# AchilleBailly/zstd-decompressor

Measured on AMD Instinct MI355X. Metric: decompressed MB/s (bit-exact vs ref) + % HBM roofline, higher is better.
Workload: dtype u8; 1 GPU; C4: enwik-style text, 128 KiB frames, zstd -3, 1 GiB unique x10 = one 10 GiB corpus; frames_total=81920, frames_rank0=81920, decompressed_bytes_total=10737418240, decompressed_bytes_rank0=10737418240, compressed_bytes_rank0=4645362830, sequences_rank0=1186360140, parallelism=replicas x1, step=zd_decode_async over every resident frame, launched per step

## Files before the change

### zstd-decompressor_amd/csrc/zd_kernels.hip

```cpp
#include <hip/hip_runtime.h>
#include <stddef.h>
#include <stdint.h>
#include <type_traits>

#include "../../include/zd.h"
#include "zd_chain.h"
#include "zd_common.h"
#include "zd_huf.h"
#include "zd_launch.h"
#include "zd_walk.h"

namespace zd {

const char* const kKernelNames[N_KERNELS] = {"zd_k_rawcopy", "zd_k_tables", "zd_k_huffman", "zd_k_sequences",
                                             "zd_k_execute", "zd_k_jexec"};
const char* const kDomNames[N_DOM] = {"zd_k_rawcopy", "zd_k_fused", "zd_k_execute", "zd_k_execute_lds",
                                      "zd_k_jsum+zd_k_jsum_blocks+zd_k_jprefix+zd_k_jscatter+zd_k_jround"};

__constant__ uint32_t c_ml_base[53] = {
    3,  4,  5,  6,  7,  8,  9,  10, 11, 12, 13, 14, 15, 16, 17, 18, 19, 20, 21, 22, 23, 24, 25, 26, 27, 28, 29,
    30, 31, 32, 33, 34, 35, 37, 39, 41, 43, 47, 51, 59, 67, 83, 99, 131, 259, 515, 1027, 2051, 4099, 8195, 16387, 32771, 65539};
__constant__ uint8_t c_ml_bits[53] = {0, 0, 0, 0, 0, 0, 0, 0, 0, 0, 0, 0, 0, 0, 0, 0, 0, 0, 0, 0, 0, 0, 0, 0, 0, 0, 0,
                                      0, 0, 0, 0, 0, 1, 1, 1, 1, 2, 2, 3, 3, 4, 4, 5, 7, 8, 9, 10, 11, 12, 13, 14, 15, 16};
__constant__ uint32_t c_ll_base[36] = {0,  1,  2,  3,  4,  5,  6,   7,   8,   9,   10,   11,   12,   13,   14,   15,   16,    18,
// ... 1504 lines not shown
                                                           uint32_t n_list, const uint16_t* __restrict__ fses,
                                                           uint64_t* __restrict__ recs) {
  __shared__ __attribute__((aligned(16))) uint16_t tabs[K3_LANES * K3_TAB];
  const int lane = threadIdx.x;
  const uint32_t li = blockIdx.x * K3_LANES + lane;
  bool act = li < n_list;
  const uint32_t ci = act ? list[li] : 0;
  CompBlock C;
  if (act) C = comp[ci];
  if (act) {
    const uint64_t key0 = fstate[C.frame].key;
    if (key0 != KEY_NONE && key_phase(key0) == PH_PARSE) act = false;
  }
  int al[3] = {0, 0, 0};
  const uint16_t* g[3] = {nullptr, nullptr, nullptr};
  if (act) {
    for (int k = 0; k < 3; k++) {
      const uint32_t s = (uint32_t)C.tab_src[k];
      al[k] = cstate[s].al[k];
      g[k] = fses + (uint64_t)comp[s].fse_slot * FSE_SLOT + k * FSE_TAB;
    }
  }
  const bool deep = act && al[1] > 8;
  const bool use_lds = __ballot(deep) == 0;
  lds_u16* mine = (lds_u16*)tabs + lane * K3_TAB;
  if (use_lds && act) {
    const int dst[3] = {0, K3_TL + K3_TM, K3_TL};
    for (int k = 0; k < 3; k++) {
      const int cnt = 1 << al[k];
      if (cnt >= 8) {
        typedef uint32_t u32x4 __attribute__((ext_vector_type(4)));
        typedef __attribute__((address_space(1))) const u32x4 g_u4;
        typedef __attribute__((address_space(3))) u32x4 l_u4;
        g_u4* s4 = (g_u4*)g[k];
        l_u4* d4 = (l_u4*)(mine + dst[k]);
        for (int e = 0; e < cnt / 8; e++) {
          u32x4 v = s4[e];
          v.x = K3_ENTRY(v.x & 0xFFFF, k, al[k]) | (K3_ENTRY(v.x >> 16, k, al[k]) << 16);
          v.y = K3_ENTRY(v.y & 0xFFFF, k, al[k]) | (K3_ENTRY(v.y >> 16, k, al[k]) << 16);
          v.z = K3_ENTRY(v.z & 0xFFFF, k, al[k]) | (K3_ENTRY(v.z >> 16, k, al[k]) << 16);
          v.w = K3_ENTRY(v.w & 0xFFFF, k, al[k]) | (K3_ENTRY(v.w >> 16, k, al[k]) << 16);
          d4[e] = v;
        }
      } else {
        for (int e = 0; e < cnt; e++) mine[dst[k] + e] = (uint16_t)K3_ENTRY(((g_u16*)g[k])[e], k, al[k]);
      }
    }
  }
  __syncthreads();
  if (!act) return;
  const CompState cs = cstate[ci];
  const uint8_t* blk = src + C.src;
  const uintptr_t lo = (uintptr_t)src;
  int st = 0;
  bool exact = !use_lds;
  if (use_lds)
    exact = K3_FAST(blk + cs.bs_off, cs.bs_size, lo, mine, mine + K3_TL, mine + K3_TL + K3_TM, al[0], al[1],
                       al[2], C.nseq, recs + C.seq_out) != 0;
  if (exact)
    st = K3_CHAIN<g_u16*, true>(blk + cs.bs_off, cs.bs_size, lo, (g_u16*)g[0], (g_u16*)g[2], (g_u16*)g[1], al[0],
                                 al[1], al[2], C.nseq, recs + C.seq_out);
  if (st) k3_fail(C, ci, cstate, fstate, st);
}
template <int CTRL>
__device__ inline uint32_t qdpp(uint32_t x) {
  return (uint32_t)__builtin_amdgcn_mov_dpp((int)x, CTRL, 0xf, 0xf, false);
}
constexpr int QP_SWAP1 = 0xB1;
constexpr int QP_SWAP2 = 0x4E;
__device__ inline uint32_t quad_sum(uint32_t x) {
  x += qdpp<QP_SWAP1>(x);
  return x + qdpp<QP_SWAP2>(x);
}
__device__ inline uint32_t quad_or(uint32_t x) {
  x |= qdpp<QP_SWAP1>(x);
  return x | qdpp<QP_SWAP2>(x);
}
__device__ inline uint32_t quad_max(uint32_t x) {
  x = max(x, qdpp<QP_SWAP1>(x));
  return max(x, qdpp<QP_SWAP2>(x));
}
template <int L, int N, bool PUB = false>
__device__ int seq_chainq(const uint8_t* bs, uint32_t bs_size, uintptr_t base, const lds_u16* tab, int role,
                          int all, int alo, int alm, uint32_t n, uint64_t* __restrict__ out,
                          volatile __attribute__((address_space(3))) uint32_t* prog = nullptr) {
  constexpr int U = (L % 2 == 0) ? L : 2 * L;
  if (bs_size == 0) return 1;
  const uint8_t lastb = bs[bs_size - 1];
  if (lastb == 0) return 1;
  int32_t pos = (int32_t)(8 * (bs_size - 1)) + highbit32(lastb);
  const int32_t A = all + alo + alm;
  if (A > pos) return 1;
  if ((intptr_t)bs - (intptr_t)base + (intptr_t)bs_size < 4 * N) return 1;
  const int32_t m = (int32_t)max((intptr_t)base - (intptr_t)bs, (intptr_t)(-4 * N));
  const int32_t pos0 = pos;
  const Win6 wi = win6_load(bs, m, pos);
  const uint32_t v0 = win6_bits(wi, pos, (uint32_t)A);
  const int alr = role == 0 ? alo : role == 1 ? alm : all;
  const uint32_t m3 = role == 3 ? 0u : ~0u, m0 = role == 0 ? 0u : ~0u;
  const uint32_t ar = (uint32_t)(alr - 31), Tr = 1u << alr;
  uint32_t s = role == 0 ? __builtin_amdgcn_ubfe(v0, alm, alo)
             : role == 1 ? __builtin_amdgcn_ubfe(v0, 0, alm)
             : v0 >> (alo + alm);
  pos -= A;
  uint32_t pS = s, pPos = (uint32_t)pos;
  auto pair_word = [&](uint32_t sB, uint32_t posB) -> uint32_t {
    const uint32_t d = pS | (sB << 10);
    const uint32_t x = d | ((pPos - posB) << 20);
    return role == 3 ? pPos : (role == 0 ? x : d);
  };
  g_u32* const outw = (g_u32*)out + role;
  const uint32_t n_even = (n + 1) & ~1u;
  WinN<N> w[L];
#pragma unroll
  for (int k = 0; k < L; k++) {
    w[k] = winn_load<N>(bs, m, k == 0 ? pos0 : pos);
    if (!(k & 1)) {
      asm volatile("" ::: "memory");
      outw[0] = pair_word(s, (uint32_t)pos);
    }
  }
  uint32_t mx = 0;
  int32_t ymin = 0;
  auto step = [&](WinN<N>& use) {
    const uint32_t e = tab[s];
    mx = max(mx, e);
    const uint32_t ns = e & 1023, nb = __builtin_clz(ns) + ar;
    const uint32_t c = e >> 10;
    const uint32_t csum = qdpp<0x00>(c) + qdpp<0x55>(c) + qdpp<0xAA>(c);
    const int32_t y = (pos - use.wb) - (int32_t)csum;
    pos -= (int32_t)csum;
    ymin = min(ymin, y);
    const uint32_t r = winn_at_tree<N>(use, (uint32_t)y);
    use = winn_load<N>(bs, m, pos);
    const uint32_t t = qdpp<0x50>(nb) & m0;
    const uint32_t v = __builtin_amdgcn_ubfe(r, t + qdpp<0x50>(t), nb);
    s = (ns << nb) + v - Tr;
  };
  uint32_t i = 0;
  g_u32* wp = outw;
  for (; i + 1 < n; i += U) {
#pragma unroll
    for (int k = 0; k < U; k += 2) {
      step(w[k % L]);
      asm volatile("" ::: "memory");
      const uint32_t slot = i + k;
      if constexpr (U == 4) {
        *wp = pair_word(s, (uint32_t)pos);
        wp += 4;
      } else {
        outw[2 * (slot < n ? slot : n_even)] = pair_word(s, (uint32_t)pos);
      }
      if constexpr (PUB) {
        constexpr int K3_PAIR_VMEM = 2 * (N / 4 + (N % 4 == 2 ? 1 : 0)) + 1;
        static_assert(7 * K3_PAIR_VMEM > 32, "seq_chainq PUB: vmcnt(32) would not cover the published line's stores");
        if (((slot + 2) & 15) == 0 && slot + 2 >= 32) {
          asm volatile("s_waitcnt vmcnt(32)" ::: "memory");
          if (role == 0) *prog = (slot + 2 - 16) >> 4;
        }
      }
      step(w[(k + 1) % L]);
      pS = s;
      pPos = (uint32_t)pos;
    }
  }
  outw[2 * (i < n ? i : n_even)] = pair_word(pS, pPos);
  const uint64_t rl = k3_reread(out, n - 1);
  const int32_t pl = (int32_t)(uint32_t)rl;
  const uint32_t st = (uint32_t)(rl >> 32);
  const uint32_t shr = role == 0 ? 20 : role == 1 ? 10 : 0;
  const uint32_t el = tab[(st >> shr) & 1023] & m3;
  mx = quad_max(max(mx, el));
  const uint32_t S = quad_sum((__builtin_clz(el & 1023) + ar) & m3);
  const int32_t E = (int32_t)(quad_sum(el >> 10) - S);
  return (mx >= K3F_BAD || ymin < 0 || pl < 0 || E > pl) ? 1 : 0;
}

#ifndef ZD_K3H_RING
#define ZD_K3H_RING 3
#endif
#ifndef ZD_K3H_DELAY
#define ZD_K3H_DELAY 1
#endif
#ifndef ZD_K3H_BITS
#define ZD_K3H_BITS 26
#endif
template <int R, int D>
__device__ constexpr int k3h_reload(int t) {
  const int x = t - 1 - D + (t - 1 - D < 0 ? 2 * R : 0);
  return x % 2 == 0 ? (x / 2) % R : -1;
}
template <int R, int D, int N>
__device__ int seq_chainqh(const uint8_t* bs, uint32_t bs_size, uintptr_t base, const lds_u16* tab, int role,
                           int all, int alo, int alm, uint32_t n, uint64_t* __restrict__ out) {
  static_assert(R >= 2 && D >= 0 && D <= 2 * R - 4, "seq_chainqh: a slot is loaded at least a whole step before its use");
  constexpr int U = 2 * R;
  if (bs_size == 0) return 1;
  const uint8_t lastb = bs[bs_size - 1];
  if (lastb == 0) return 1;
  int32_t pos = (int32_t)(8 * (bs_size - 1)) + highbit32(lastb);
  const int32_t A = all + alo + alm;
  if (A > pos) return 1;
  if ((intptr_t)bs - (intptr_t)base + (intptr_t)bs_size < 4 * N) return 1;
  const int32_t m = (int32_t)max((intptr_t)base - (intptr_t)bs, (intptr_t)(-4 * N));
  const Win6 wi = win6_load(bs, m, pos);
  const uint32_t v0 = win6_bits(wi, pos, (uint32_t)A);
  const int alr = role == 0 ? alo : role == 1 ? alm : all;
  const uint32_t m3 = role == 3 ? 0u : ~0u, m0 = role == 0 ? 0u : ~0u;
  const uint32_t ar = (uint32_t)(alr - 31), Tr = 1u << alr;
  uint32_t s = role == 0 ? __builtin_amdgcn_ubfe(v0, alm, alo)
             : role == 1 ? __builtin_amdgcn_ubfe(v0, 0, alm)
             : v0 >> (alo + alm);
  pos -= A;
  uint32_t pS = s, pPos = (uint32_t)pos;
  auto pair_word = [&](uint32_t sB, uint32_t posB) -> uint32_t {
    const uint32_t d = pS | (sB << 10);
    const uint32_t x = d | ((pPos - posB) << 20);
    return role == 3 ? pPos : (role == 0 ? x : d);
  };
  g_u32* const outw = (g_u32*)out + role;
  const uint32_t n_even = (n + 1) & ~1u;
  WinN<N> w[R];
  w[0] = winn_load<N>(bs, m, pos);
  asm volatile("" ::: "memory");
  outw[0] = pair_word(s, (uint32_t)pos);
#pragma unroll
  for (int k = 1; k < R; k++) w[k] = w[0];
  uint32_t mx = 0;
  int32_t ymin = 0;
  auto step = [&](WinN<N>& use, WinN<N>* rl) {
    const uint32_t e = tab[s];
    mx = max(mx, e);
    const uint32_t ns = e & 1023, nb = __builtin_clz(ns) + ar;
    const uint32_t c = e >> 10;
    const uint32_t csum = qdpp<0x00>(c) + qdpp<0x55>(c) + qdpp<0xAA>(c);
    const int32_t y = (pos - use.wb) - (int32_t)csum;
    pos -= (int32_t)csum;
    ymin = min(ymin, y);
    uint32_t r = winn_at_tree<N>(use, (uint32_t)y);
    if (rl) {
      if (rl == &use) asm volatile("" : "+v"(r) : : "memory");
      *rl = winn_load<N>(bs, m, pos);
    }
    const uint32_t t = qdpp<0x50>(nb) & m0;
    const uint32_t v = __builtin_amdgcn_ubfe(r, t + qdpp<0x50>(t), nb);
    s = (ns << nb) + v - Tr;
  };
  uint32_t i = 0;
  g_u32* wp = outw;
  for (; i + 1 < n; i += U) {
#pragma unroll
    for (int k = 0; k < R; k++) {
      const int ra = k3h_reload<R, D>(2 * k), rb = k3h_reload<R, D>(2 * k + 1);
      step(w[k], ra >= 0 ? &w[ra] : nullptr);
      asm volatile("" ::: "memory");
      if (k < 2)
        wp[4 * k] = pair_word(s, (uint32_t)pos);
      else
        outw[2 * min(i + 2 * k, n_even)] = pair_word(s, (uint32_t)pos);
      step(w[k], rb >= 0 ? &w[rb] : nullptr);
      pS = s;
      pPos = (uint32_t)pos;
    }
    wp += 4 * R;
  }
  outw[2 * (i < n ? i : n_even)] = pair_word(pS, pPos);
  const uint64_t rl = k3_reread(out, n - 1);
  const int32_t pl = (int32_t)(uint32_t)rl;
  const uint32_t st = (uint32_t)(rl >> 32);
  const uint32_t shr = role == 0 ? 20 : role == 1 ? 10 : 0;
  const uint32_t el = tab[(st >> shr) & 1023] & m3;
  mx = quad_max(max(mx, el));
  const uint32_t S = quad_sum((__builtin_clz(el & 1023) + ar) & m3);
  const int32_t E = (int32_t)(quad_sum(el >> 10) - S);
  return (mx >= K3F_BAD || ymin < 0 || pl < 0 || E > pl) ? 1 : 0;
}

#ifdef ZD_K3_COUNT
__device__ unsigned long long zd_k3_count[4];
extern "C" int zd_debug_k3_count(unsigned long long* v, int reset) {
  if (hipMemcpyFromSymbol(v, HIP_SYMBOL(zd_k3_count), sizeof(zd_k3_count)) != hipSuccess) return -1;
  if (reset) {
    const unsigned long long z[4] = {0, 0, 0, 0};
    if (hipMemcpyToSymbol(HIP_SYMBOL(zd_k3_count), z, sizeof(z)) != hipSuccess) return -1;
  }
  return 0;
}
#endif

#ifndef ZD_K3Q_CHAINS
#define ZD_K3Q_CHAINS 16
#endif
constexpr int K3Q_CHAINS = ZD_K3Q_CHAINS;
static_assert(K3Q_CHAINS == 8 || K3Q_CHAINS == 16, "K3Q: 8 or 16 chains per wave");
__global__ __launch_bounds__(64) void zd_k_sequences_q(const uint8_t* __restrict__ src,
                                                       const CompBlock* __restrict__ comp, CompState* cstate,
                                                       FrameState* fstate, const uint32_t* __restrict__ list,
                                                       uint32_t n_list, const uint16_t* __restrict__ fses,
                                                       uint64_t* __restrict__ recs, const uint8_t* __restrict__ redo) {
  __shared__ __attribute__((aligned(16))) uint16_t tabs[K3Q_CHAINS * K3_TAB];
  const int lane = threadIdx.x;
  const int role = lane & 3, q = lane >> 2;
  const uint32_t li = blockIdx.x * K3Q_CHAINS + q;
  bool act = q < K3Q_CHAINS && li < n_list;
  const uint32_t ci = act ? list[li] : 0;
  CompBlock C;
  if (act) C = comp[ci];
  if (act && redo && !redo[C.frame]) act = false;
  if (act) {
    const uint64_t key0 = fstate[C.frame].key;
    if (key0 != KEY_NONE && key_phase(key0) == PH_PARSE) act = false;
  }
  int al[3] = {0, 0, 0};
  const uint16_t* g[3] = {nullptr, nullptr, nullptr};
  if (act) {
    for (int k = 0; k < 3; k++) {
      const uint32_t sidx = (uint32_t)C.tab_src[k];
      al[k] = cstate[sidx].al[k];
      g[k] = fses + (uint64_t)comp[sidx].fse_slot * FSE_SLOT + k * FSE_TAB;
    }
  }
  const bool deep = act && al[1] > 8;
  const bool use_lds = __ballot(deep) == 0;
  lds_u16* mine = (lds_u16*)tabs + q * K3_TAB;
  if (use_lds && act) {
    const int dst[3] = {0, K3_TL + K3_TM, K3_TL};
    if (role < 3) {
      const int k = role;
      const int cnt = 1 << al[k];
      if (cnt >= 8) {
        typedef uint32_t u32x4 __attribute__((ext_vector_type(4)));
        typedef __attribute__((address_space(1))) const u32x4 g_u4;
        typedef __attribute__((address_space(3))) u32x4 l_u4;
        g_u4* s4 = (g_u4*)g[k];
        l_u4* d4 = (l_u4*)(mine + dst[k]);
        for (int e = 0; e < cnt / 8; e++) {
          u32x4 v = s4[e];
          v.x = K3_ENTRY(v.x & 0xFFFF, k, al[k]) | (K3_ENTRY(v.x >> 16, k, al[k]) << 16);
          v.y = K3_ENTRY(v.y & 0xFFFF, k, al[k]) | (K3_ENTRY(v.y >> 16, k, al[k]) << 16);
          v.z = K3_ENTRY(v.z & 0xFFFF, k, al[k]) | (K3_ENTRY(v.z >> 16, k, al[k]) << 16);
          v.w = K3_ENTRY(v.w & 0xFFFF, k, al[k]) | (K3_ENTRY(v.w >> 16, k, al[k]) << 16);
          d4[e] = v;
        }
      } else {
        for (int e = 0; e < cnt; e++) mine[dst[k] + e] = (uint16_t)K3_ENTRY(((g_u16*)g[k])[e], k, al[k]);
      }
    }
  }
  __syncthreads();
  if (!act) return;
  const CompState cs = cstate[ci];
  const uint8_t* blk = src + C.src;
  const uintptr_t lo = (uintptr_t)src;
  int st = 0;
  bool exact = !use_lds;
  if (use_lds) {
    const lds_u16* tab = role == 0 ? mine + K3_TL + K3_TM : role == 1 ? mine + K3_TL : mine;
    const bool half = ZD_K3H_BITS > 0 && __ballot(8ull * cs.bs_size > (uint64_t)ZD_K3H_BITS * C.nseq) == 0;
    if (half)
      exact = seq_chainqh<ZD_K3H_RING, ZD_K3H_DELAY, ZD_K3_WN>(blk + cs.bs_off, cs.bs_size, lo, tab, role, al[0], al[1], al[2],
                                                 C.nseq, recs + C.seq_out) != 0;
    else
      exact = seq_chainq<ZD_K3_LA, ZD_K3_WN>(blk + cs.bs_off, cs.bs_size, lo, tab, role, al[0], al[1], al[2], C.nseq,
                                            recs + C.seq_out) != 0;
#ifdef ZD_K3_COUNT
    if (role == 0) {
      atomicAdd(&zd_k3_count[0], 1ull);
      if (half) atomicAdd(&zd_k3_count[1], 1ull);
      if (exact) atomicAdd(&zd_k3_count[half ? 3 : 2], 1ull);
    }
#endif
  }
  if (exact && role == 0)
    st = K3_CHAIN<g_u16*, true>(blk + cs.bs_off, cs.bs_size, lo, (g_u16*)g[0], (g_u16*)g[2], (g_u16*)g[1], al[0],
                                 al[1], al[2], C.nseq, recs + C.seq_out);
  if (st) k3_fail(C, ci, cstate, fstate, st);
}
constexpr uint32_t K3L_ML = 4096, K3L_OF = 8192, K3L_BYTES = 10240;
#ifndef ZD_K3L_ASM
#define ZD_K3L_ASM 1
#endif
#ifndef ZD_K3L_SHADOW
#define ZD_K3L_SHADOW 1
#endif
typedef __attribute__((address_space(3))) uint64_t lds_u64;
typedef __attribute__((address_space(3))) uint32_t lds_u32;
__device__ inline uint64_t k3l_entry(uint32_t e, int k, int al, uint32_t tab) {
  const uint32_t c = e & 63, ns = (e >> 6) & 1023;
  uint32_t base, eb;
  bool bad;
  if (k == 0) { ll_code(c, &base, &eb); bad = c > 35; }
  else if (k == 2) { ml_code(c, &base, &eb); bad = c > 52; }
  else { eb = c; bad = c > 31; }
  bad = bad || ns == 0 || hb32(ns) > al;
  const uint32_t nb = bad ? 0u : (uint32_t)(al - hb32(ns));
  const uint32_t bl = bad ? 0u : (ns << nb) - (1u << al);
  const uint32_t lo = bad ? (1u << 16) : (nb | ((eb + nb) << 8));
  return (uint64_t)lo | ((uint64_t)(tab + 8 * bl) << 32);
}
__device__ inline void k3l_tables(const uint16_t* __restrict__ fses, const CompBlock& C, const CompBlock* __restrict__ comp,
                                  const CompState* __restrict__ cstate, uint32_t tb, int al[3], int lane) {
  for (int k = 0; k < 3; k++) {
    const uint32_t s = (uint32_t)C.tab_src[k];
    al[k] = cstate[s].al[k];
    const uint16_t* g = fses + (uint64_t)comp[s].fse_slot * FSE_SLOT + k * FSE_TAB;
    const uint32_t t = tb + (k == 0 ? 0u : k == 2 ? K3L_ML : K3L_OF);
    const int cnt = 1 << min(al[k], k == 1 ? 8 : 9);
    for (int e = lane; e < cnt; e += 64) *(lds_u64*)(uintptr_t)(t + 8 * e) = k3l_entry(g[e], k, al[k], t);
  }
}
template <bool PUB = false>
__device__ int seq_chainl(const uint8_t* bs, uint32_t bs_size, uintptr_t base, uint32_t tb, int all, int alo, int alm,
                          uint32_t n, uint64_t* __restrict__ out, volatile lds_u32* prog = nullptr) {
  const int lane = threadIdx.x & 63;
  if (bs_size == 0 || (tb & 4095) || alo > 8) return 1;
  const uint8_t lastb = bs[bs_size - 1];
  if (lastb == 0) return 1;
  int32_t pos = (int32_t)(8 * (bs_size - 1)) + highbit32(lastb);
  const int32_t A = all + alo + alm;
  if (A > pos) return 1;
  const uint8_t* bsa = (const uint8_t*)((uintptr_t)bs & ~(uintptr_t)3);
  const int32_t boff = (int32_t)(((uintptr_t)bs & 3) * 8);
  const uint64_t below = ((uintptr_t)bsa - (base & ~(uintptr_t)3)) >> 2;
  const int32_t dmin = below > (1u << 30) ? -(1 << 30) : -(int32_t)below;
  auto wload = [&](int32_t D) -> uint32_t {
    const int32_t d = max(D + lane, dmin);
    return *(const g_u32*)(bsa + 4 * (int64_t)d);
  };
  int32_t D = ((pos + boff) >> 5) - 62;
  int32_t Q = pos + boff - 32 * D;
  int32_t qb = 32 * D - boff;
  auto shl1 = [](uint32_t w) { return (uint32_t)__builtin_amdgcn_update_dpp(0, (int)w, 0x130, 0xf, 0xf, false); };
  uint32_t win = wload(D);
  uint32_t win1 = shl1(win);
  uint32_t nxt;
  auto bits32 = [&](int32_t q) -> uint32_t {
    int32_t qd;
    asm("v_ashrrev_i32 %0, 5, %1" : "=v"(qd) : "v"(q));
    const int idx = __builtin_amdgcn_readfirstlane(qd);
    const uint32_t lo = (uint32_t)__builtin_amdgcn_readlane((int)win, idx);
    const uint32_t hi = (uint32_t)__builtin_amdgcn_readlane((int)win1, idx);
#if ZD_K3L_ASM
    uint64_t r;
    asm("v_lshrrev_b64 %0, %1, %2" : "=v"(r) : "v"((uint32_t)q & 31u), "s"(((uint64_t)hi << 32) | lo));
    return (uint32_t)r;
#else
    return (uint32_t)((((uint64_t)hi << 32) | lo) >> (q & 31));
#endif
  };
  const uint32_t v0 = bits32(Q - A) & (uint32_t)((1ull << A) - 1);
  uint32_t aL = tb + 8 * (v0 >> (alo + alm));
  uint32_t aO = tb + K3L_OF + 8 * __builtin_amdgcn_ubfe(v0, alm, alo);
  uint32_t aM = tb + K3L_ML + 8 * __builtin_amdgcn_ubfe(v0, 0, alm);
  Q -= A;
  uint32_t bad = 0;
#ifdef ZD_K3L_PROF
  const uint64_t tp0 = __builtin_amdgcn_s_memtime();
  const uint64_t rp0 = __builtin_amdgcn_s_memrealtime();
#endif
  auto lshl3_add = [](uint32_t v, uint32_t b) -> uint32_t {
    uint32_t r;
    asm("v_lshl_add_u32 %0, %1, 3, %2" : "=v"(r) : "v"(v), "v"(b));
    return r;
  };
  uint64_t eL, eM, eO;
  auto issue = [&]() {
    eL = *(const lds_u64*)(uintptr_t)aL;
    eM = *(const lds_u64*)(uintptr_t)aM;
    eO = *(const lds_u64*)(uintptr_t)aO;
  };
  auto finish = [&]() {
    const uint32_t lL = (uint32_t)eL, lM = (uint32_t)eM, lO = (uint32_t)eO;
    const uint32_t lOM = lO + lM;
#if ZD_K3L_ASM
    uint32_t ls;
    asm("v_add3_u32 %0, %1, %2, %3" : "=v"(ls) : "v"(lO), "v"(lM), "v"(lL));
#else
    const uint32_t ls = lOM + lL;
#endif
    bad |= ls;
    Q -= (ls >> 8) & 255;
    const uint32_t r = bits32(Q);
    const uint32_t vO = __builtin_amdgcn_ubfe(r, 0, lO), vM = __builtin_amdgcn_ubfe(r, lO, lM);
    const uint32_t vL = __builtin_amdgcn_ubfe(r, lOM, lL);
    aO = lshl3_add(vO, (uint32_t)(eO >> 32));
    aM = lshl3_add(vM, (uint32_t)(eM >> 32));
    aL = lshl3_add(vL, (uint32_t)(eL >> 32));
  };
  auto step = [&]() { issue(); finish(); };
  auto sx = [](uint32_t a) { return __builtin_amdgcn_ubfe(a, 3, 9); };
  auto put = [&](uint64_t* p, uint32_t pA, uint32_t lA, uint32_t mA, uint32_t oA, uint32_t pB, uint32_t lB, uint32_t mB,
                 uint32_t oB) {
#ifdef ZD_EXP_K3L_RAWPUT
    *(g_u32x4g*)p = u32x4g{oA, mA, lA, pA};
    asm volatile("" ::: "memory");
    *(g_u32x4g*)p = u32x4g{oB, mB, lB, pB};
#else
    const u32x4g v{sx(oA) | (sx(oB) << 10) | ((pA - pB) << 20), sx(mA) | (sx(mB) << 10), sx(lA) | (sx(lB) << 10), pA};
    *(g_u32x4g*)p = v;
#endif
  };
  const uint32_t n_even = (n + 1) & ~1u;
  uint32_t pP = (uint32_t)(Q + qb), pL = aL, pM = aM, pO = aO;
  uint32_t i = 0;
  uint64_t* wp = out;
  while (i + 1 < n) {
  if (__builtin_amdgcn_readfirstlane(Q >> 5) < 13) {
    D -= 48;
    Q += 48 * 32;
    qb -= 48 * 32;
    win = nxt;
    win1 = shl1(win);
  }
  nxt = wload(D - 48);
  do {
#pragma unroll
    for (int k = 0; k < 4; k += 2) {
      step();
#if ZD_K3L_SHADOW
      uint32_t cP = (uint32_t)(Q + qb), cL = aL, cM = aM, cO = aO;
      issue();
      asm volatile("" : "+v"(pP), "+v"(pL), "+v"(pM), "+v"(pO), "+v"(cP), "+v"(cL), "+v"(cM), "+v"(cO) :: "memory");
      put(wp, pP, pL, pM, pO, cP, cL, cM, cO);
      wp += 2;
      finish();
#else
      put(wp, pP, pL, pM, pO, (uint32_t)(Q + qb), aL, aM, aO);
      wp += 2;
      step();
#endif
      pP = (uint32_t)(Q + qb); pL = aL; pM = aM; pO = aO;
    }
    i += 4;
    if constexpr (PUB) {
      if ((i & 15) == 0 && i >= 32) {
        asm volatile("s_waitcnt vmcnt(8)" ::: "memory");
        if (lane == 0) *prog = (i - 16) >> 4;
      }
    }
  } while (i + 1 < n && __builtin_amdgcn_readfirstlane(Q >> 5) >= 13);
  }
  put(out + (i < n ? i : n_even), pP, pL, pM, pO, pP, pL, pM, pO);
#ifdef ZD_K3L_PROF
  {
    const uint64_t tp1 = __builtin_amdgcn_s_memtime(), rp1 = __builtin_amdgcn_s_memrealtime();
    if (lane == 0 && blockIdx.x < 4)
      printf("K3L block %u: %u steps, %.1f memtime ticks a step, %.1f ns a step (memrealtime 100 MHz)\n", blockIdx.x, i,
             (double)(tp1 - tp0) / (double)max(i, 1u), 10.0 * (double)(rp1 - rp0) / (double)max(i, 1u));
  }
#endif
  asm volatile("s_waitcnt vmcnt(0)" ::: "memory");
  const uint64_t rl = k3_reread(out, n - 1);
  const int32_t pl = (int32_t)(uint32_t)rl;
  const uint32_t st = (uint32_t)(rl >> 32);
  const uint32_t lL = *(const lds_u32*)(uintptr_t)(tb + 8 * (st & 1023));
  const uint32_t lM = *(const lds_u32*)(uintptr_t)(tb + K3L_ML + 8 * ((st >> 10) & 1023));
  const uint32_t lO = *(const lds_u32*)(uintptr_t)(tb + K3L_OF + 8 * ((st >> 20) & 255));
  const uint32_t ls = lL + lM + lO;
  const int32_t E = (int32_t)(((ls >> 8) & 255) - ((lL & 31) + (lM & 31) + (lO & 31)));
#ifdef ZD_EXP_K3L_RAWPUT
  return 1;
#endif
  return ((bad | ls) >> 16 || pl < 0 || E > pl) ? 1 : 0;
}

__global__ __launch_bounds__(64) void zd_k_sequences_l(const uint8_t* __restrict__ src,
                                                       const CompBlock* __restrict__ comp, CompState* cstate,
                                                       FrameState* fstate, const uint32_t* __restrict__ list,
                                                       uint32_t n_list, const uint16_t* __restrict__ fses,
                                                       uint64_t* __restrict__ recs, const uint8_t* __restrict__ redo) {
  __shared__ __attribute__((aligned(4096))) uint64_t tabs[K3L_BYTES / 8];
  const int lane = threadIdx.x;
  const uint32_t li = blockIdx.x;
  if (li >= n_list) return;
  const uint32_t ci = list[li];
  const CompBlock C = comp[ci];
  if (redo && !redo[C.frame]) return;
  const uint64_t key0 = fstate[C.frame].key;
  if (key0 != KEY_NONE && key_phase(key0) == PH_PARSE) return;
  const uint32_t tb = (uint32_t)(uintptr_t)(__attribute__((address_space(3))) uint64_t*)tabs;
  int al[3];
  k3l_tables(fses, C, comp, cstate, tb, al, lane);
  __syncthreads();
  const CompState cs = cstate[ci];
  const uint8_t* blk = src + C.src;
  int st = 0;
  if (seq_chainl(blk + cs.bs_off, cs.bs_size, (uintptr_t)src, tb, al[0], al[1], al[2], C.nseq, recs + C.seq_out) &&
      lane == 0) {
    const uint16_t* g[3];
    for (int k = 0; k < 3; k++) {
      const uint32_t s = (uint32_t)C.tab_src[k];
      g[k] = fses + (uint64_t)comp[s].fse_slot * FSE_SLOT + k * FSE_TAB;
    }
    st = K3_CHAIN<g_u16*, true>(blk + cs.bs_off, cs.bs_size, (uintptr_t)src, (g_u16*)g[0], (g_u16*)g[2], (g_u16*)g[1],
                                al[0], al[1], al[2], C.nseq, recs + C.seq_out);
  }
  if (st) k3_fail(C, ci, cstate, fstate, st);
}

__device__ inline uint64_t rec_lane(uint64_t raw, int lane) {
  const uint32_t lo = (uint32_t)raw, hi = (uint32_t)(raw >> 32);
  const uint32_t plo = qdpp<QP_SWAP1>(lo), phi = qdpp<QP_SWAP1>(hi);
  const uint32_t h = lane & 1;
  return rec_unpack(h ? plo : lo, h ? phi : hi, h ? lo : plo, h ? hi : phi, h);
}

#ifndef ZD_K4_W
#define ZD_K4_W 4096
#endif
#ifndef ZD_K4_B
#define ZD_K4_B 1536
#endif
constexpr int K4_W = ZD_K4_W;
constexpr int K4_B = ZD_K4_B;
#ifndef ZD_K4_C
#define ZD_K4_C 7200
#endif
constexpr int K4_C = ZD_K4_C;
typedef uint32_t u32x4 __attribute__((ext_vector_type(4)));
typedef uint32_t u32x4a1 __attribute__((ext_vector_type(4), aligned(1)));
typedef __attribute__((address_space(3))) uint8_t l_u8;
typedef __attribute__((address_space(3))) u32x4a1 l_u32x4a1;
typedef __attribute__((address_space(3))) uint64_t l_u64a1 __attribute__((aligned(1)));
typedef __attribute__((address_space(3))) uint32_t l_u32a1 __attribute__((aligned(1)));
typedef __attribute__((address_space(3))) uint16_t l_u16a1 __attribute__((aligned(1)));
typedef __attribute__((address_space(1))) const u32x4a1 g_cu32x4a1;
typedef __attribute__((address_space(1))) u32x4 g_u32x4;
typedef __attribute__((address_space(3))) u32x4 l_u32x4;

__device__ inline u32x4 ldg16(const uint8_t* p) { return *(g_cu32x4a1*)p; }
__device__ inline u32x4 ldg16_src(const uint8_t* p) { return *(g_cu32x4a1*)p; }
__device__ inline u32x4 ldg16_once(const uint8_t* p) {
  return *(g_cu32x4a1*)p;
}
__device__ inline u32x4 lds16(const l_u8* p) { return *(const l_u32x4a1*)p; }
__device__ inline void sts_n(l_u8* p, u32x4 v, uint32_t n) {
  if (n >= 16) { *(l_u32x4a1*)p = v; return; }
  if (n & 8) { *(l_u64a1*)p = (uint64_t)v.x | ((uint64_t)v.y << 32); v.x = v.z; v.y = v.w; p += 8; }
  if (n & 4) { *(l_u32a1*)p = v.x; v.x = v.y; p += 4; }
  if (n & 2) { *(l_u16a1*)p = (uint16_t)v.x; v.x >>= 16; p += 2; }
  if (n & 1) { *p = (uint8_t)v.x; }
}
__device__ inline void wait_vm() { asm volatile("s_waitcnt vmcnt(0)" ::: "memory"); }
__device__ inline uint32_t period16(uint32_t off) {
  constexpr uint64_t T = 16ull | 16ull << 5 | 18ull << 10 | 16ull << 15 | 20ull << 20 | 18ull << 25 | 21ull << 30;
  return off >= 8 ? 2 * off : (uint32_t)(T >> (5 * ((off - 1) & 7))) & 31;
}
__device__ inline int64_t readlane_i64(int64_t x, int l) {
  int lo = __shfl((int)(uint32_t)x, l, 64);
  int hi = __shfl((int)(uint32_t)((uint64_t)x >> 32), l, 64);
  return (int64_t)(((uint64_t)(uint32_t)hi << 32) | (uint32_t)lo);
}

__device__ inline uint64_t readlane_any_u64(uint64_t x, int l) {
// ... 3560 lines not shown
```

Measured before the change: 331,500 MB/s.

## Cooperatively load FSE tables into LDS across the whole wave

Replaces the per-chain table fill, where only three lanes of each chain copied their table serially, with a wave-wide cooperative load. Slot and accuracy-log descriptors are broadcast with readlane, and all 64 lanes fetch 16-byte chunks for 8 chains at a time before converting them into LDS. It also hoists the CompState load and the metadata loads ahead of the activity checks, so those global reads can overlap. The cost is more registers for the staged vectors and loads issued for inactive or small tables, which may lower occupancy.

Measured after the change: 337,500 MB/s (median of 6 runs). 1.8% higher.

```diff
diff --git a/zstd-decompressor_amd/csrc/zd_kernels.hip b/zstd-decompressor_amd/csrc/zd_kernels.hip
--- a/zstd-decompressor_amd/csrc/zd_kernels.hip
+++ b/zstd-decompressor_amd/csrc/zd_kernels.hip
@@ -1830,54 +1830,89 @@
   const int lane = threadIdx.x;
   const int role = lane & 3, q = lane >> 2;
   const uint32_t li = blockIdx.x * K3Q_CHAINS + q;
-  bool act = q < K3Q_CHAINS && li < n_list;
-  const uint32_t ci = act ? list[li] : 0;
+  const bool act0 = q < K3Q_CHAINS && li < n_list;
+  bool act = act0;
+  const uint32_t ci = act0 ? list[li] : 0;
   CompBlock C;
-  if (act) C = comp[ci];
-  if (act && redo && !redo[C.frame]) act = false;
-  if (act) {
+  CompState cs;
+  int al[3] = {0, 0, 0};
+  uint32_t slot[3] = {0, 0, 0};
+  if (act0) {
+    C = comp[ci];
     const uint64_t key0 = fstate[C.frame].key;
-    if (key0 != KEY_NONE && key_phase(key0) == PH_PARSE) act = false;
-  }
-  int al[3] = {0, 0, 0};
-  const uint16_t* g[3] = {nullptr, nullptr, nullptr};
-  if (act) {
+    cs = cstate[ci];
     for (int k = 0; k < 3; k++) {
       const uint32_t sidx = (uint32_t)C.tab_src[k];
       al[k] = cstate[sidx].al[k];
-      g[k] = fses + (uint64_t)comp[sidx].fse_slot * FSE_SLOT + k * FSE_TAB;
-    }
-  }
+      slot[k] = comp[sidx].fse_slot;
+    }
+    if (redo && !redo[C.frame]) act = false;
+    if (key0 != KEY_NONE && key_phase(key0) == PH_PARSE) act = false;
+  }
+  const uint16_t* g[3];
+  for (int k = 0; k < 3; k++) g[k] = fses + (uint64_t)slot[k] * FSE_SLOT + k * FSE_TAB;
   const bool deep = act && al[1] > 8;
   const bool use_lds = __ballot(deep) == 0;
   lds_u16* mine = (lds_u16*)tabs + q * K3_TAB;
-  if (use_lds && act) {
-    const int dst[3] = {0, K3_TL + K3_TM, K3_TL};
-    if (role < 3) {
-      const int k = role;
-      const int cnt = 1 << al[k];
-      if (cnt >= 8) {
-        typedef uint32_t u32x4 __attribute__((ext_vector_type(4)));
-        typedef __attribute__((address_space(1))) const u32x4 g_u4;
-        typedef __attribute__((address_space(3))) u32x4 l_u4;
-        g_u4* s4 = (g_u4*)g[k];
-        l_u4* d4 = (l_u4*)(mine + dst[k]);
-        for (int e = 0; e < cnt / 8; e++) {
-          u32x4 v = s4[e];
-          v.x = K3_ENTRY(v.x & 0xFFFF, k, al[k]) | (K3_ENTRY(v.x >> 16, k, al[k]) << 16);
-          v.y = K3_ENTRY(v.y & 0xFFFF, k, al[k]) | (K3_ENTRY(v.y >> 16, k, al[k]) << 16);
-          v.z = K3_ENTRY(v.z & 0xFFFF, k, al[k]) | (K3_ENTRY(v.z >> 16, k, al[k]) << 16);
-          v.w = K3_ENTRY(v.w & 0xFFFF, k, al[k]) | (K3_ENTRY(v.w >> 16, k, al[k]) << 16);
-          d4[e] = v;
-        }
-      } else {
-        for (int e = 0; e < cnt; e++) mine[dst[k] + e] = (uint16_t)K3_ENTRY(((g_u16*)g[k])[e], k, al[k]);
-      }
+  if (use_lds) {
+    typedef uint32_t u32x4 __attribute__((ext_vector_type(4)));
+    typedef __attribute__((address_space(1))) const u32x4 g_u4;
+    typedef __attribute__((address_space(3))) u32x4 l_u4;
+    constexpr int QR = 8;
+    const uint32_t desc = act ? (uint32_t)al[0] | (uint32_t)al[1] << 8 | (uint32_t)al[2] << 16 | 1u << 24 : 0u;
+    auto conv = [](u32x4 v, int k, int a) -> u32x4 {
+      v.x = K3_ENTRY(v.x & 0xFFFF, k, a) | (K3_ENTRY(v.x >> 16, k, a) << 16);
+      v.y = K3_ENTRY(v.y & 0xFFFF, k, a) | (K3_ENTRY(v.y >> 16, k, a) << 16);
+      v.z = K3_ENTRY(v.z & 0xFFFF, k, a) | (K3_ENTRY(v.z >> 16, k, a) << 16);
+      v.w = K3_ENTRY(v.w & 0xFFFF, k, a) | (K3_ENTRY(v.w >> 16, k, a) << 16);
+      return v;
+    };
+    const int hl = lane >> 5, l32 = lane & 31;
+#pragma unroll 1
+    for (int h = 0; h < K3Q_CHAINS; h += QR) {
+      u32x4 vl[QR], vm[QR], vo[QR / 2];
+#pragma unroll
+      for (int j = 0; j < QR; j++) {
+        const uint32_t s0 = (uint32_t)__builtin_amdgcn_readlane((int)slot[0], 4 * (h + j));
+        const uint32_t s2 = (uint32_t)__builtin_amdgcn_readlane((int)slot[2], 4 * (h + j));
+        vl[j] = ((g_u4*)(fses + (uint64_t)s0 * FSE_SLOT))[lane];
+        vm[j] = ((g_u4*)(fses + (uint64_t)s2 * FSE_SLOT + 2 * FSE_TAB))[lane];
+      }
+#pragma unroll
+      for (int j = 0; j < QR; j += 2) {
+        const uint32_t sa = (uint32_t)__builtin_amdgcn_readlane((int)slot[1], 4 * (h + j));
+        const uint32_t sb = (uint32_t)__builtin_amdgcn_readlane((int)slot[1], 4 * (h + j + 1));
+        vo[j / 2] = ((g_u4*)(fses + (uint64_t)(hl ? sb : sa) * FSE_SLOT + FSE_TAB))[l32];
+      }
+      asm volatile("" : "+v"(vl[0]));
+#pragma unroll
+      for (int j = 0; j < QR; j++) {
+        const uint32_t d = (uint32_t)__builtin_amdgcn_readlane((int)desc, 4 * (h + j));
+        const int a0 = d & 255, a2 = (d >> 16) & 255;
+        const int on = d >> 24;
+        lds_u16* t = (lds_u16*)tabs + (h + j) * K3_TAB;
+        if (on && a0 >= 3 && 8 * lane < (1 << a0)) ((l_u4*)t)[lane] = conv(vl[j], 0, a0);
+        if (on && a2 >= 3 && 8 * lane < (1 << a2)) ((l_u4*)(t + K3_TL))[lane] = conv(vm[j], 2, a2);
+      }
+#pragma unroll
+      for (int j = 0; j < QR; j += 2) {
+        const uint32_t da = (uint32_t)__builtin_amdgcn_readlane((int)desc, 4 * (h + j));
+        const uint32_t db = (uint32_t)__builtin_amdgcn_readlane((int)desc, 4 * (h + j + 1));
+        const uint32_t d = hl ? db : da;
+        const int a1 = (d >> 8) & 255;
+        lds_u16* t = (lds_u16*)tabs + (h + j + hl) * K3_TAB + K3_TL + K3_TM;
+        if ((d >> 24) && a1 >= 3 && 8 * l32 < (1 << a1)) ((l_u4*)t)[l32] = conv(vo[j / 2], 1, a1);
+      }
+    }
+    const int ar = role == 0 ? al[0] : role == 1 ? al[1] : al[2];
+    if (act && role < 3 && ar < 3) {
+      const int dst = role == 0 ? 0 : role == 1 ? K3_TL + K3_TM : K3_TL;
+      const g_u16* gr = (g_u16*)(role == 0 ? g[0] : role == 1 ? g[1] : g[2]);
+      for (int e = 0; e < (1 << ar); e++) mine[dst + e] = (uint16_t)K3_ENTRY(gr[e], role, ar);
     }
   }
   __syncthreads();
   if (!act) return;
-  const CompState cs = cstate[ci];
   const uint8_t* blk = src + C.src;
   const uintptr_t lo = (uintptr_t)src;
   int st = 0;
```
